# siyarvurucu/gym-macm

Hardware: AMD Instinct MI355X
Metric: agent·steps/sec, cm-flock-v0 64 agents × 4096 envs, at 1/2/4/8 MI355X (higher is better)
Workload: dtype f32; 1 GPU; cm-flock-v0 n_agents=[64] x 4096 envs per GPU, uniform random discrete actions (MultiDiscrete[3,3,3]) pre-generated on device, from reset (seed 0x6d61636d); envs_per_gpu=4096, n_agents=64, total_envs=4096, split=weak: 4096 envs per GPU, parallelism=env-sharded x1 (no data-path collective), obs=float32, max_contacts=2016, spill_slots=4096, launch=one macm_world_rollout_traj launch for the K timed steps, outputs=every step's ([K, E, N, ...] trajectory buffers)

## Files before the change

gym-macm_amd/csrc/flock_common.hpp:

```cpp
#pragma once

#include <hip/hip_runtime.h>
#include <stdint.h>

#include "../../include/macm.h"
#include "macm_math.h"

namespace macm {

constexpr float kEps = 1.1920928955078125e-07f;
constexpr float kLinearSlop = 0.005f;
constexpr float kAabbExtension = 0.1f;
constexpr float kAabbMultiplier = 2.0f;
constexpr float kMaxTranslation = 2.0f;
constexpr float kBaumgarte = 0.2f;
constexpr float kMaxLinearCorrection = 0.2f;
constexpr float kTimeToSleep = 0.5f;
constexpr float kLinearSleepTol = 0.01f;
constexpr float kPi32 = 3.14159265359f;

struct StepParams {
  int32_t n_envs, n_agents, n_targets, max_contacts;
  int32_t vel_iters, pos_iters, warm_starting;
  int32_t action_mode, reward_mode, coord;
  int32_t force_spill;
  int32_t sweep;
  float dt;
  float inv_dt;
  float inv_mass;
  float damp;
  float radius;
  float friction;
  float force_f32;
  double rot_step;
  double inv_hz;
  double force;
  double diag_c;
  double reward_radius;
  double time_limit;
};

struct WorldBuffers {
  float2* pos;
  float2* vel;
  float* angle;
  float4* fat;
  float* sleep;
  float2* targets;
// ... 126 lines not shown
  int2* listener;
  int32_t* winner;
  uint8_t* mask_out;
  double* health_out;
  uint8_t* alive_out;
  int32_t* winner_out;
  float4* snap_out;
};

__host__ __device__ inline int tdm_team_of(const TdmParams& T, int i) {
  int t = 0;
  while (t < T.n_teams - 1 && i >= T.team_end[t]) ++t;
  return t;
}

__device__ __forceinline__ void act_trig(float a, double* s0, double* c0, double* s1, double* c1) {
  if (fabsf(a) < 524288.0f) {
    macm_action_trig(a, s0, c0, s1, c1);
  } else {
    sincos((double)a, s0, c0);
    sincos((double)a + M_PI / 2, s1, c1);
  }
}

template <typename OT>
__device__ __forceinline__ double obs_sqrt(float x) {
  if constexpr (sizeof(OT) == 4) return (double)sqrtf(x);
  else return sqrt((double)x);
}

__device__ __forceinline__ float rcp_rn(float x) {
  const float y = __builtin_amdgcn_rcpf(x);
  const float e = __builtin_fmaf(-x, y, 1.0f);
// ... 144 lines not shown
```

gym-macm_amd/csrc/flock_rollout_ar_w64.hip:

```cpp
#define MACM_ROLLOUT_TU 1
#define MACM_AUTORESET_TU 1
#include "flock_step_w64.hip"
```

gym-macm_amd/csrc/flock_rollout_w64.hip:

```cpp
#define MACM_ROLLOUT_TU 1
#include "flock_step_w64.hip"
```

gym-macm_amd/csrc/flock_step_w64.hip:

```cpp
#include "bots.hpp"
#include "flock_common.hpp"
#include "flock_spill.hpp"
#include "tdm_obs.hpp"

namespace macm {

constexpr int W = 64;
constexpr int TCAP = 256;
constexpr int DEG = 16;
constexpr int ICAP = W / 2;
constexpr int RCH = 2;
constexpr int KREC = 4;
constexpr int KRECA = KREC;
constexpr int kLevelsMinIsland = 4;
constexpr int kPrio2T = 3;

#if defined(MACM_STAMPS) && !defined(MACM_TIMELINE)
#define STAMP(k)                                                                    \
  do {                                                                              \
    __builtin_amdgcn_s_waitcnt(0);                                                  \
    const unsigned long long _t = __builtin_amdgcn_s_memtime();                     \
    if (lane == 0) B.stamps[(size_t)e * 16 + (k)] = _t;                             \
  } while (0)
#define STAMP_STAT(k, v)                                                            \
// ... 62 lines not shown
  if (coord == MACM_COORD_CARTESIAN) {
    o[0] = (OT)r0;
    o[1] = (OT)cos(t0);
    o[2] = (OT)sin(t0);
    o[3] = (OT)r1;
    o[4] = (OT)cos(t1);
    o[5] = (OT)sin(t1);
  } else if constexpr (sizeof(OT) == 4) {
    st_g<kOut>(reinterpret_cast<float4*>(o), make_float4((float)r0, (float)t0, (float)r1, (float)t1));
  } else {
    st_g<kOut>(reinterpret_cast<double2*>(o), make_double2(r0, t0));
    st_g<kOut>(reinterpret_cast<double2*>(o) + 1, make_double2(r1, t1));
  }
}

template <typename OT>
__device__ __forceinline__ void write_obs(OT* o, int coord, float ang, float best, float rx, float ry, float tdx,
                                          float tdy, float td2) {
  const double t0 = wrap_pi(obs_atan2((double)ry, (double)rx) - (double)ang);
  const double t1 = wrap_pi(obs_atan2((double)tdy, (double)tdx) - (double)ang);
  write_obs_row(o, coord, obs_sqrt<OT>(best), t0, obs_sqrt<OT>(td2), t1);
}

typedef float pf2 __attribute__((ext_vector_type(2)));

__device__ __forceinline__ void warm_start_contact_pk(pf2& vA, pf2& vB, float nx, float ny, float ln, float ltg,
                                                      float mA, float mB) {
  const pf2 n = {nx, ny}, t = {ny, -nx};
  const pf2 P = ln * n + ltg * t;
  vA = vA - mA * P;
  vB = vB + mB * P;
}

__device__ __forceinline__ void solve_velocity_contact_pk(pf2& vA, pf2& vB, float nx, float ny, float& ln,
                                                          float& ltg, float mA, float mB, float kmass,
// ... 400 lines not shown
  }
  near2_min<2 * K, 32 + 2 * K, SCAL>(qa.x, qa.y, qb.x, qb.y, cme, st);
  near2_min<2 * K + 1, 33 + 2 * K, SCAL>(qa.z, qa.w, qb.z, qb.w, cme, st);
  if constexpr ((K & 1) == 1) __builtin_amdgcn_sched_barrier(0);
  if constexpr (K + 1 < 16) near2_step<K + 1, SCAL>(s_pc2, win, cme, st);
}

constexpr float kNearS = 1.0f;
constexpr int kNearCap = 12;
constexpr int kNearRetry = 8, kNearRetryMax = 64;
constexpr float kNearPad = 1.0f + 0x1p-18f;
constexpr float kNearMove2 = (kNearS * 0.25f) * (kNearS * 0.25f) * (1.0f - 0x1p-20f);
constexpr int kNearNone = 0, kNearValid = 1, kNearDense = 2;
constexpr int kNearCtlKeep = 1;
constexpr int kNearCtlPlain = 2;
constexpr int kNearKindPlain = 0, kNearKindList = 1, kNearKindRebuild = 2;

__device__ __forceinline__ void near_push(float d2, float thr2, uint32_t& mask) {
  asm volatile(
      "v_cmp_le_f32 vcc, %1, %2\n\t"
      "v_addc_co_u32 %0, vcc, %0, %0, vcc"
      : "+v"(mask)
      : "v"(d2), "v"(thr2)
      : "vcc");
}

__device__ __forceinline__ unsigned long long near_build(const float4* s_pc2, fvec2 cme, float thr2) {
  uint32_t lo = 0u, hi = 0u;
  float4 na = s_pc2[15], nb = s_pc2[31];
#pragma unroll 4
// ... 49 lines not shown
  return row;
}

__device__ __forceinline__ int write_new_pairs(int lane, unsigned long long newmask, uint32_t* ocab,
                                               float2* ocimp, int C, uint32_t* stage_ab = nullptr,
                                               float2* stage_im = nullptr) {
  const int cnt = __popcll(newmask);
  const int pre = wave_prefix_sum(cnt);
  const int total = __builtin_amdgcn_readlane(pre, W - 1);
  int w = total - pre;
  unsigned long long m = newmask;
  while (m) {
    const int j = 63 - __clzll(m);
    m &= ~(1ull << j);
    if (w < C) {
      st_g<kState>(ocab + w, (uint32_t)lane | ((uint32_t)j << 16));
      st_g<kState>(ocimp + w, make_float2(0.0f, 0.0f));
      if (stage_ab && w < RCH * W) {
        stage_ab[w] = (uint32_t)lane | ((uint32_t)j << 16);
        stage_im[w] = make_float2(0.0f, 0.0f);
      }
    }
    ++w;
  }
  return total;
}

struct TailObs {
  unsigned long long* ctl;
  unsigned int tag;
  int nsteps;
  int k;
  bool worker;
  bool more;
  int q, left;
// ... 84 lines not shown
  }
  __syncthreads();
}

struct StepCarry {
  bool valid;
  float2 p, v, tg;
  float ang, slp;
  float4 fat;
  uint32_t rab[RCH];
  float2 rim[RCH];
  uint32_t ar0, ar1;
  int M, step_count;
};

template <int MODE, int NCAP, typename OT, bool SCAL = false, bool CARRY = false, bool NEARL = false>
__device__ __attribute__((always_inline)) inline void step_w64_body(
    const StepParams& P, const WorldBuffers& B, const TdmParams& TP, const TdmBuffers& TB, int cur,
    const void* __restrict__ actions, OT* __restrict__ obs, int32_t* __restrict__ nbr_out,
    float* __restrict__ rew_out, uint8_t* __restrict__ coll_out, uint8_t* __restrict__ done_out,
    const int e = blockIdx.x, const int lane = threadIdx.x, TailObs* tl = nullptr, StepCarry* carry = nullptr,
    const void* actions_next = nullptr, void** pool_out = nullptr, const int near_ctl = 0) {
  constexpr bool kT = MODE == kTdm;
  static_assert(!CARRY || !kT, "the carried step is Flock's");
  static_assert(!NEARL || (!kT && NCAP == 64), "the candidate lists are the 64-record Flock sweep's");
#ifdef MACM_TIMELINE
  const unsigned long long tl_rt0 = __builtin_amdgcn_s_memrealtime(), tl_c0 = __builtin_amdgcn_s_memtime();
#endif
  const int N = P.n_agents;
  const int C = P.max_contacts;
  bool act = lane < N;
  const size_t ag = (size_t)e * N + lane;
  const int nxt = cur ^ 1;
  const unsigned long long lt = lanemask_lt(lane);

  __shared__ float2 s_c[W];
  __shared__ float2 s_v[W];
  constexpr int TMW = kT ? 1 : 2;
// ... 24 lines not shown
  static_assert(kT || sizeof(uint32_t) * 2 * 2 * W >= W * DEG, "s_adj must fit in s_tm");
  static_assert(sizeof(uint32_t) * 2 * TMW * W >= sizeof(float2) * W, "the level steps' dummy slots must fit in s_tm");
  __shared__ uint8_t s_ord[TCAP];
  __shared__ uint32_t s_cvis[TCAP / 32];
  __shared__ uint8_t s_deg[W], s_stack[W], s_ibodies[W], s_bisl[W];
  __shared__ uint16_t s_ic[ICAP + 1];
  __shared__ uint8_t s_ib[ICAP + 1];
  __shared__ uint8_t s_isolved[ICAP];
  __shared__ uint32_t s_imin[ICAP];
  __shared__ int s_nisl;
  __shared__ double s_hpd[W];
  __shared__ int8_t s_hit[W];
  __shared__ float s_ang[W];
  __shared__ uint4 s_nl[NEARL ? W : 1];
  __shared__ int s_nl_state, s_nl_retry;
#ifdef MACM_STAMPS
  __shared__ int s_stat_maxisl;
  int stat_near = 0;
#endif
  if constexpr (kT) {
    if (tl && tl->worker) {
      tdm_tail_row<OT>(P, B, TP, TB, obs, *tl, lane, s_c, s_ang, reinterpret_cast<float4*>(&s_pool),
                       tdm_obs_rb_stage_bytes(N) <= (int)sizeof(Pool));
      return;
    }
  }

  const uint32_t* cab = B.cab[cur] + (size_t)e * C;
  const float2* cimp = B.cimp[cur] + (size_t)e * C;
  bool carried = false;
// ... 113 lines not shown
  float ray_x = 0.0f, ray_y = 0.0f;
  if (act) {
    if (P.action_mode == MACM_ACTION_DISCRETE) {
      float af = (float)((double)ang + ((double)(a2 - 1) * P.rot_step) * P.inv_hz);
      double ad = (double)af;
      if (fabs(ad) > M_PI) {
        af = (float)(ad - sgn(ad) * (2.0 * M_PI));
        ad = (double)af;
      }
      ang = af;
      const double cc = ((a0 != 1) && (a1 != 1)) ? P.diag_c : 1.0;
      const double k0 = (double)(a0 - 1), k1 = (double)(a1 - 1);
      double force = P.force;
      if constexpr (kT) force = P.force * (1.0 - TP.percent_mov_penalty * (double)(cdm > 0.0));
      double s0, c0, s1, c1;
      act_trig(af, &s0, &c0, &s1, &c1);
      const double fx = (c0 * k0 + c1 * k1) * cc * force;
      const double fy = (s0 * k0 + s1 * k1) * cc * force;
      Fx = (float)fx;
      Fy = (float)fy;
      if constexpr (kT) {
        if (cda <= 0.0) {
          if (a3) {
            attacking = true;
            ray_x = p.x + (float)(TP.melee_range * c0);
            ray_y = p.y + (float)(TP.melee_range * s0);
            cda = TP.cooldown_atk;
            cdm = TP.cooldown_mov_penalty;
          }
        } else {
          cda -= P.inv_hz;
// ... 135 lines not shown
      if (TMW == 2 && T > 64) tmask1 = (unsigned long long)tm[2] | ((unsigned long long)tm[3] << 32);
      deg = __popcll(tmask) + __popcll(tmask1);
    }
  } else if (act) {
    for (int t = 0; t < T; ++t) {
      const uint32_t ab = s_tab[t];
      if ((int)(ab & 0xffffu) == lane || (int)(ab >> 16) == lane) {
        if (deg < DEG) s_adj[lane * DEG + deg] = (uint8_t)t;
        ++deg;
      }
    }
  }
  if constexpr (!kT) {
    if (touch_over || (!fast_dfs && __builtin_amdgcn_ballot_w64(deg > DEG) != 0ull) || P.force_spill) {
      if constexpr (CARRY) {
        if (carried) __builtin_amdgcn_fence(__ATOMIC_SEQ_CST, "workgroup");
        carry->valid = false;
      }
      if constexpr (NEARL) s_nl_state = kNearNone;
      spill::step_env<OT, true>(P, B, e, cur, actions, obs, nbr_out, rew_out, coll_out, done_out,
                                reinterpret_cast<unsigned char*>(&s_pool));
      return;
    }
  } else {
    if (touch_over || (!fast_dfs && __builtin_amdgcn_ballot_w64(deg > DEG) != 0ull) || P.force_spill) {
      __shared__ int s_slot;
      const int slot = spill::acquire_slot(B, e, &s_slot);
      if (slot < 0) {
        spill::keep_lists(P, B, e, cur);
        if (lane == 0) {
          B.status[e] |= MACM_ST_SPILL_WAIT;
// ... 691 lines not shown
      float4 win[kNearAhead];
#pragma unroll
      for (int k = 0; k < kNearAhead; ++k) win[k] = s_pc2[k];
      near_step<0, NCAP>(s_pc2, win, mk2(cx, cy), s1);
      best = s1.best;
      bj = s1.bj;
    }
  }
  const unsigned long long myov = moved_pairs(movedm, fn, lane) & valid & ~(1ull << lane);
  const unsigned long long oldm = (unsigned long long)s_oldm[2 * lane] | ((unsigned long long)s_oldm[2 * lane + 1] << 32);
  const bool coll = act && ((myov | oldm) != 0ull);
  const unsigned long long above = lane == 63 ? 0ull : (~0ull << (lane + 1));
  const unsigned long long newmask = act ? (myov & ~oldm & above) : 0ull;
  STAMP(10);

  if constexpr (CARRY) {
    if (lane == 0) {
      time_passed = B.time_passed[e];
      st_prev = B.status[e];
      const ulonglong2* ec = reinterpret_cast<const ulonglong2*>(B.env_counters + (size_t)e * 4);
      const ulonglong2 c01 = ec[0], c23 = ec[1];
      ctr[0] = c01.x;
      ctr[1] = c01.y;
      ctr[2] = c23.x;
      ctr[3] = c23.y;
    }
  }
  uint32_t* ocab = B.cab[nxt] + (size_t)e * C;
  float2* ocimp = B.cimp[nxt] + (size_t)e * C;
  uint32_t* const stage_ab = CARRY ? s_tab : nullptr;
  float2* const stage_im = CARRY ? reinterpret_cast<float2*>(s_tm) : nullptr;
  static_assert(sizeof(uint32_t) * RCH * W <= sizeof(s_pool.tab), "the staged entries must fit in s_tab");
  static_assert(!CARRY || sizeof(float2) * RCH * W <= sizeof(s_pool.tm), "the staged impulses must fit in s_tm");
  const int nnew = write_new_pairs(lane, newmask, ocab, ocimp, C, stage_ab, stage_im);
  int kept = 0, Tr = 0;
  for (int c = 0; c * W < M; ++c) {
    const int k = c * W + lane;
    uint32_t ab = 0u;
    if (c < RCH) {
#pragma unroll
      for (int q = 0; q < RCH; ++q)
// ... 5 lines not shown
    const bool touch = (tbits >> c) & 1u;
    if (k < M) {
      const int a = ab & 0xffffu, b = ab >> 16;
      keep = overlap(s_fn[a], s_fn[b]);
    }
    const unsigned long long mt = __ballot(touch), mk = __ballot(keep);
    const int trank = Tr + __popcll(mt & lt);
    const int krank = kept + __popcll(mk & lt);
    Tr += __popcll(mt);
    kept += __popcll(mk);
    if (keep) {
      const int w = nnew + krank;
      if (w < C) {
        float2 l = make_float2(0.0f, 0.0f);
        if (touch && trank < TCAP) l = make_float2(s_tln[trank], s_tlt[trank]);
        st_g<kState>(ocab + w, ab);
        st_g<kState>(ocimp + w, l);
        if constexpr (CARRY) {
          if (w < RCH * W) {
            stage_ab[w] = ab;
            stage_im[w] = l;
          }
        }
      }
    }
  }
  int total = nnew + kept;
  if (total > C) {
    status |= MACM_ST_CONTACT_OVERFLOW;
    total = C;
  }
  STAMP(11);

  float rew = 0.0f;
  if constexpr (!kT) {
    if (act) {
      const float tdx = tg.x - cx, tdy = tg.y - cy;
      const float td2 = tdx * tdx + tdy * tdy;
      const double d = sqrt((double)td2);
      if (coll) rew = -1.0f;
      else if (P.reward_mode == MACM_REWARD_LINEAR) rew = (float)((-d / 35) + 1);
      else rew = (d < P.reward_radius) ? 1.0f : 0.0f;
      st_g<kOut>(rew_out + ag, rew);
      if (coll_out) st_g<kOut>(coll_out + ag, (uint8_t)(coll ? 1 : 0));
      if (nbr_out) st_g<kOut>(nbr_out + ag, (int32_t)bj);
      if (obs) {
        const int od = P.coord == MACM_COORD_CARTESIAN ? 6 : 4;
        const float2 cn = s_c[bj];
        const float rx = cn.x - cx, ry = cn.y - cy;
        write_obs<OT>(obs + ag * od, P.coord, ang, best, rx, ry, tdx, tdy, td2);
      }
      st_g<kState>(B.pos + ag, make_float2(cx, cy));
      st_g<kState>(B.vel + ag, make_float2(vx, vy));
      st_g<kState>(B.angle + ag, ang);
      st_g<kState>(B.fat + ag, fn);
      st_g<kState>(B.sleep + ag, ns);
    }
  } else {
    if (lane < N) {
      if (act) {
        B.pos[ag] = make_float2(cx, cy);
        B.vel[ag] = make_float2(vx, vy);
        B.fat[ag] = fn;
        B.sleep[ag] = ns;
      }
      if (act0) {
        B.angle[ag] = ang;
        TB.cd_atk[ag] = cda;
        TB.cd_mov[ag] = cdm;
      }
      TB.health[ag] = hp;
// ... 31 lines not shown
  if constexpr (!kT) {
    c1 = __popcll(__ballot(act && coll));
    c2 = __popcll(__ballot(act && rew > 0.0f));
    if (P.reward_mode == MACM_REWARD_LINEAR) rsum = wave_pairwise_sum((double)rew);
  } else {
    c1 = __popcll(att_m);
    c2 = __popcll(alive0_m & ~livem);
    const int myteam = tdm_team_of(TP, lane);
    for (int t = 0; t < TP.n_teams; ++t)
      if (__ballot(act && myteam == t)) {
        ++alive_teams;
        last_team = t;
      }
  }
  if (lane == 0) {
    const double tp = time_passed + P.inv_hz;
    uint8_t dn = tp > P.time_limit ? 1 : 0;
    if constexpr (kT) {
      int win = win_prev;
      if (done_prev) dn = 1;
      if (alive_teams == 1) {
        dn = 1;
        win = last_team;
      }
      if (alive_teams == 0) dn = 1;
      TB.winner[e] = win;
      if (TB.winner_out) TB.winner_out[e] = win;
      TB.listener[e] = lis;
    }
    B.time_passed[e] = tp;
    B.done[e] = dn;
    if (done_out) done_out[e] = dn;
    B.step_count[e] = step_count + 1;
    B.ccount[nxt][e] = total;
    const int st = (mst1 ? 1 : 0) | (mst2 ? 2 : 0) | (mst4 ? 4 : 0);
    if (st) {
      B.status[e] = st_prev | st;
      report_status(B, st);
    }
    const unsigned long long c0 = kT ? (unsigned long long)__popcll(alive0_m) : (unsigned long long)N;
    ulonglong2* ec = reinterpret_cast<ulonglong2*>(B.env_counters + (size_t)e * 4);
    ec[0] = make_ulonglong2(ctr[0] + c0, ctr[1] + c1);
    ec[1] = make_ulonglong2(ctr[2] + c2, ctr[3] + (unsigned long long)dn);
    if constexpr (!kT) {
      if (P.reward_mode == MACM_REWARD_LINEAR) add_reward_sum(B, e, rsum);
    }
  }
  if constexpr (CARRY) {
    carry->p = make_float2(cx, cy);
    carry->v = make_float2(vx, vy);
    carry->ang = ang;
    carry->fat = fn;
    carry->slp = ns;
    carry->tg = tg;
    carry->M = total;
    carry->step_count = step_count + 1;
    __syncthreads();
#pragma unroll
    for (int c = 0; c < RCH; ++c) {
      const int k = c * W + lane;
      carry->rab[c] = 0u;
      carry->rim[c] = make_float2(0.0f, 0.0f);
      if (k < total) {
        carry->rab[c] = stage_ab[k];
        carry->rim[c] = stage_im[k];
      }
    }
    carry->valid = total <= RCH * W && !(mst1 | mst2 | mst4);
  }
  if constexpr (NEARL) {
    if (mst1 | mst2 | mst4) s_nl_state = kNearNone;
  }
  STAMP(13);
#ifdef MACM_TIMELINE
  {
    const unsigned long long rt1 = __builtin_amdgcn_s_memrealtime(), c1t = __builtin_amdgcn_s_memtime();
    const unsigned long long hw = (unsigned)__builtin_amdgcn_s_getreg((31 << 11) | 4);
    const unsigned long long xcc = (unsigned)__builtin_amdgcn_s_getreg((31 << 11) | 20);
    if (lane == 0) {
      unsigned long long* st = B.stamps + (size_t)e * 16;
// ... 229 lines not shown
    if constexpr (MODE == kTdm) {
      TB.mask_out = traj_row(TB.mask_out, kr, EN * (N - 1));
      TB.health_out = traj_row(TB.health_out, kr, EN);
      TB.alive_out = traj_row(TB.alive_out, kr, EN);
      TB.winner_out = traj_row(TB.winner_out, kr, (size_t)A.P.n_envs);
      TB.snap_out = A.tail_tag ? (k >= A.tail_k0 ? traj_row(TB.snap_out, (size_t)(k - A.tail_k0), EN) : nullptr)
                               : traj_row(TB.snap_out, kr, EN);
    }
    const size_t abytes = MODE == kTdm ? 4 : 3;
    uint8_t* const pol_in = A.policy_act ? A.policy_act + kr * EN * abytes : nullptr;
    __builtin_amdgcn_s_setprio(0);
    int sl = (int)threadIdx.x;
    if constexpr (MODE == kTdm) asm volatile("" : "+v"(sl));
    tl.k = k - A0.tail_k0;
    constexpr bool kNearL = MODE == kFlock && NCAP == 64;
    const int near_ctl = kNearL ? (k > 0 ? kNearCtlKeep : 0) | ((A.cur & kRollNearPlainBit) ? kNearCtlPlain : 0) : 0;
    if constexpr (CARRY) {
      const unsigned char* const act_k = static_cast<const unsigned char*>(A.actions) + (size_t)k * A.astride;
      step_w64_body<MODE, NCAP, OT, SCAL, true, kNearL>(
          A.P, A.B, A.TP, TB, (A.cur ^ k) & 1, act_k, obs, traj_row(A.nbr_out, kr, EN), traj_row(A.rew_out, kr, EN),
          traj_row(A.coll_out, kr, EN), traj_row(A.done_out, kr, (size_t)A.P.n_envs), env, sl, nullptr, &cy,
          k + 1 < ksteps ? act_k + A.astride : nullptr, nullptr, near_ctl);
      if (A.cur & kRollReloadBit) cy.valid = false;
      if (!cy.valid) __builtin_amdgcn_fence(__ATOMIC_SEQ_CST, "workgroup");
      __syncthreads();
    } else {
      step_w64_body<MODE, NCAP, OT, SCAL, false, kNearL>(
          A.P, A.B, A.TP, TB, kNearL ? (A.cur ^ k) & 1 : A.cur ^ (k & 1),
          pol_in ? pol_in : static_cast<const unsigned char*>(A.actions) + (size_t)k * A.astride, obs,
          traj_row(A.nbr_out, kr, EN), traj_row(A.rew_out, kr, EN), traj_row(A.coll_out, kr, EN),
          traj_row(A.done_out, kr, (size_t)A.P.n_envs), env, sl, MODE == kTdm ? &tl : nullptr, nullptr, nullptr, nullptr,
// ... 371 lines not shown
```

gym-macm_amd/csrc/macm_capi.hip:

```cpp
#include <math.h>
#include <stdio.h>
#include <string.h>

#include <algorithm>
#include <string>
#include <vector>

#include "flock_common.hpp"
#include "py_mt19937.hpp"

namespace macm {
hipError_t launch_step_w64(const StepParams& P, const WorldBuffers& B, int cur, const void* actions, void* obs,
                           bool obs_f64, int32_t* nbr, float* rew, uint8_t* coll, uint8_t* done, hipStream_t s);
hipError_t launch_rollout_w64(const StepParams& P, const WorldBuffers& B, int cur, const void* actions, void* obs,
                              bool obs_f64, int32_t* nbr, float* rew, uint8_t* coll, uint8_t* done, hipStream_t s,
                              int nsteps, unsigned long long astride, int traj, int reload);
hipError_t launch_init_w64(const StepParams& P, const WorldBuffers& B, int cur, void* obs, bool obs_f64,
                           int32_t* nbr, const uint8_t* mask, hipStream_t s);
hipError_t launch_observe_w64(const StepParams& P, const WorldBuffers& B, void* obs, bool obs_f64, int32_t* nbr,
                              hipStream_t s);
hipError_t launch_step_wg(const StepParams& P, const WorldBuffers& B, int cur, int tcap, const void* actions,
                          void* obs, bool obs_f64, int32_t* nbr, float* rew, uint8_t* coll, uint8_t* done,
                          hipStream_t s, HandoffStream* HS, uint8_t* bot_act = nullptr);
hipError_t launch_init_wg(const StepParams& P, const WorldBuffers& B, int cur, void* obs, bool obs_f64, int32_t* nbr,
// ... 383 lines not shown
  P.n_envs = n_envs;
  P.n_agents = N;
  P.n_targets = T;
  P.max_contacts = C;
  P.vel_iters = c.velocity_iterations;
  P.pos_iters = c.position_iterations;
  P.warm_starting = c.warm_starting ? 1 : 0;
  P.action_mode = c.action_mode;
  P.reward_mode = c.reward_mode;
  P.coord = c.coord;
  P.force_spill = 0;
  P.sweep = 0;
  fill_body_params(P, c.hz, c.radius, c.density, c.friction, c.linear_damping, c.agent_force,
                   c.agent_rotation_speed);
  P.reward_radius = c.reward_radius;
  P.time_limit = c.time_limit;

  WorldBuffers& B = w->B;
  memset(&B, 0, sizeof(B));
  const size_t EN = (size_t)n_envs * N;
  int rc = MACM_OK;
  if ((rc = dalloc(w, &B.pos, EN)) || (rc = dalloc(w, &B.vel, EN)) || (rc = dalloc(w, &B.angle, EN)) ||
      (rc = dalloc(w, &B.fat, EN)) || (rc = dalloc(w, &B.sleep, EN)) ||
      (rc = dalloc(w, &B.targets, (size_t)n_envs * T)) || (rc = dalloc(w, &B.tidx, (size_t)N)) ||
      (rc = dalloc(w, &B.ccount[0], (size_t)n_envs)) || (rc = dalloc(w, &B.ccount[1], (size_t)n_envs)) ||
      (rc = dalloc(w, &B.cab[0], (size_t)n_envs * C)) || (rc = dalloc(w, &B.cab[1], (size_t)n_envs * C)) ||
      (rc = dalloc(w, &B.cimp[0], (size_t)n_envs * C)) || (rc = dalloc(w, &B.cimp[1], (size_t)n_envs * C)) ||
      (rc = dalloc(w, &B.step_count, (size_t)n_envs)) || (rc = dalloc(w, &B.time_passed, (size_t)n_envs)) ||
      (rc = dalloc(w, &B.done, (size_t)n_envs)) || (rc = dalloc(w, &B.status, (size_t)n_envs)) ||
      (rc = dalloc(w, &B.env_counters, (size_t)n_envs * 4)) || (rc = dalloc(w, &B.env_rsum, (size_t)n_envs))
// ... 1418 lines not shown
```

gym-macm_amd/csrc/macm_math.h:

```cpp
#pragma once
#include <math.h>

#ifdef __HIPCC__
#define MACM_MATH_FN __device__ __forceinline__
#else
#define MACM_MATH_FN static inline
#endif

MACM_MATH_FN void macm_sincos(double x, double* sp, double* cp) {
  const double fn = rint(x * 6.36619772367581382433e-01);
  const int q = (int)fn;
  const double t1 = fma(-fn, 1.57079632673412561417e+00, x);
  const double w2 = fn * 6.07710050630396597660e-11;
  const double r2 = t1 - w2;
  const double e2 = (t1 - r2) - w2;
  const double tail = fma(-fn, 2.02226624879595063154e-21, e2);
  const double y0 = r2 + tail;
  const double y1 = (r2 - y0) + tail;
  const double z = y0 * y0;
  double ps = 1.58969099521155010221e-10;
  ps = fma(ps, z, -2.50507602534068634195e-08);
  ps = fma(ps, z, 2.75573137070700676789e-06);
  ps = fma(ps, z, -1.98412698298579493134e-04);
  ps = fma(ps, z, 8.33333333332248946124e-03);
  const double v = z * y0;
  const double s = y0 - ((z * (0.5 * y1 - v * ps) - y1) - v * -1.66666666666666324348e-01);
  double pc = -1.13596475577881948265e-11;
  pc = fma(pc, z, 2.08757232129817482790e-09);
  pc = fma(pc, z, -2.75573143513906633035e-07);
  pc = fma(pc, z, 2.48015872894767294178e-05);
  pc = fma(pc, z, -1.38888888888741095749e-03);
  pc = fma(pc, z, 4.16666666666666019037e-02);
  const double hz = 0.5 * z;
  const double wc = 1.0 - hz;
  const double c = wc + (((1.0 - wc) - hz) + (z * (z * pc) - y0 * y1));
  const int odd = q & 1;
  double so = odd ? c : s, co = odd ? s : c;
  if (q & 2) so = -so;
  if ((q + 1) & 2) co = -co;
  *sp = (x == 0.0) ? x : so;
  *cp = co;
}

MACM_MATH_FN void macm_sincos_pair(double x, double* s0p, double* c0p, double* s1p, double* c1p) {
  const double fn = rint(x * 6.36619772367581382433e-01);
  const int q = (int)fn;
  const double t1 = fma(-fn, 1.57079632673412561417e+00, x);
  const double w2 = fn * 6.07710050630396597660e-11;
  const double r2 = t1 - w2;
  const double e2 = (t1 - r2) - w2;
  const double tail = fma(-fn, 2.02226624879595063154e-21, e2);
  const double y0 = r2 + tail;
  const double y1 = (r2 - y0) + tail;
  const double P = 1.57079632679489655800e+00;
  const double x1 = x + P;
  const double bp = x1 - x;
  const double err = (x - (x1 - bp)) + (P - bp);
  const double y1b = y1 - (6.12323399573676603587e-17 + err);
  const double z = y0 * y0;
  double ps = 1.58969099521155010221e-10;
  ps = fma(ps, z, -2.50507602534068634195e-08);
  ps = fma(ps, z, 2.75573137070700676789e-06);
  ps = fma(ps, z, -1.98412698298579493134e-04);
  ps = fma(ps, z, 8.33333333332248946124e-03);
  const double v = z * y0;
  const double vs = v * -1.66666666666666324348e-01;
  const double vps = v * ps;
  const double sa = y0 - ((z * (0.5 * y1 - vps) - y1) - vs);
  const double sb = y0 - ((z * (0.5 * y1b - vps) - y1b) - vs);
  double pc = -1.13596475577881948265e-11;
  pc = fma(pc, z, 2.08757232129817482790e-09);
  pc = fma(pc, z, -2.75573143513906633035e-07);
  pc = fma(pc, z, 2.48015872894767294178e-05);
  pc = fma(pc, z, -1.38888888888741095749e-03);
  pc = fma(pc, z, 4.16666666666666019037e-02);
  const double hz = 0.5 * z;
  const double wc = 1.0 - hz;
  const double cz = ((1.0 - wc) - hz) + z * (z * pc);
  const double ca = wc + (cz - y0 * y1);
  const double cb = wc + (cz - y0 * y1b);
  const int odd = q & 1;
  double so = odd ? ca : sa, co = odd ? sa : ca;
  if (q & 2) so = -so;
  if ((q + 1) & 2) co = -co;
  const int q1 = q + 1;
  double so1 = odd ? sb : cb, co1 = odd ? cb : sb;
  if (q1 & 2) so1 = -so1;
  if ((q1 + 1) & 2) co1 = -co1;
  *s0p = (x == 0.0) ? x : so;
  *c0p = co;
  *s1p = so1;
  *c1p = co1;
}

#ifdef __cplusplus
#define MACM_MATH_TABLE static constexpr
#else
#define MACM_MATH_TABLE static const
#endif
#include "trig_fix.inc"

MACM_MATH_FN void macm_action_trig_raw(double x, double* s0, double* c0, double* s1, double* c1) {
  if (fabs(x) < 4.0) {
    macm_sincos_pair(x, s0, c0, s1, c1);
  } else {
    macm_sincos(x, s0, c0);
    macm_sincos(x + M_PI / 2, s1, c1);
  }
}

MACM_MATH_FN void macm_action_trig(float a, double* s0, double* c0, double* s1, double* c1) {
  macm_action_trig_raw((double)a, s0, c0, s1, c1);
  int hit = 0;
  for (int i = 0; i < MACM_TRIG_NNEAR; ++i) hit |= a == (float)kTrigFixNear[i][0];
  if (hit) {
    for (int i = 0; i < MACM_TRIG_NNEAR; ++i) {
      if (a == (float)kTrigFixNear[i][0]) {
        *s0 = kTrigFixNear[i][1]; *c0 = kTrigFixNear[i][2]; *s1 = kTrigFixNear[i][3]; *c1 = kTrigFixNear[i][4];
      }
    }
  }
  if (fabsf(a) >= 4.0f) {
    for (int i = 0; i < MACM_TRIG_NFAR; ++i) {
      if (a == (float)kTrigFixFar[i][0]) {
        *s0 = kTrigFixFar[i][1]; *c0 = kTrigFixFar[i][2]; *s1 = kTrigFixFar[i][3]; *c1 = kTrigFixFar[i][4];
      }
    }
  }
}

MACM_MATH_FN double obs_atan2_core(double ax, double ay) {
  const int swap = ay > ax;
  const double mx = swap ? ay : ax, mn = swap ? ax : ay;
  const int r0 = mn < 0.4375 * mx;
  const int r1 = !r0 && mn < 0.6875 * mx;
  const double ca = r1 ? 2.0 : 1.0, cb = r0 ? 0.0 : 1.0, cd = r0 ? 0.0 : 1.0;
  const double xr = fma(ca, mn, -(cb * mx)) / fma(cd, mn, ca * mx);
  const double z = xr * xr;
  double p = 1.62858201153657823623e-02;
  p = fma(p, z, -3.65315727442169155270e-02);
  p = fma(p, z, 4.97687799461593236017e-02);
  p = fma(p, z, -5.83357013379057348645e-02);
  p = fma(p, z, 6.66107313738753120669e-02);
  p = fma(p, z, -7.69187620504482999495e-02);
  p = fma(p, z, 9.09088713343650656196e-02);
  p = fma(p, z, -1.11111104054623557880e-01);
  p = fma(p, z, 1.42857142725034663711e-01);
  p = fma(p, z, -1.99999999998764832476e-01);
  p = fma(p, z, 3.33333333333329318027e-01);
  const double sz = z * p;
  const double hi = r1 ? 4.63647609000806093515e-01 : 7.85398163397448278999e-01;
  const double lo = r1 ? 2.26987774529616870924e-17 : 3.06161699786838301793e-17;
  double r = r0 ? fma(-xr, sz, xr) : hi - (fma(xr, sz, -lo) - xr);
  if (swap) r = (1.57079632679489655800e+00 - r) + 6.12323399573676603587e-17;
  return r;
}

MACM_MATH_FN double obs_atan2_finish(double r, double y, double x) {
  if (x < 0.0) r = (3.1415926535897931160e+00 - r) + 1.2246467991473531772e-16;
  if (x == 0.0 && y == 0.0) r = signbit(x) ? 3.1415926535897931160e+00 : 0.0;
  return copysign(r, y);
}

MACM_MATH_FN double obs_atan2(double y, double x) { return obs_atan2_finish(obs_atan2_core(fabs(x), fabs(y)), y, x); }
```

gym-macm_amd/csrc/rollout_autoreset.inc:

```

constexpr int kMtN = 624, kMtM = 397;

__device__ __forceinline__ uint32_t mt_temper(uint32_t y) {
  y ^= (y >> 11);
  y ^= (y << 7) & 0x9d2c5680u;
  y ^= (y << 15) & 0xefc60000u;
  y ^= (y >> 18);
  return y;
}

__device__ __forceinline__ uint32_t mt_mix(uint32_t hi, uint32_t lo, uint32_t src) {
  const uint32_t y = (hi & 0x80000000u) | (lo & 0x7fffffffu);
  return src ^ (y >> 1) ^ ((y & 1u) ? 0x9908b0dfu : 0u);
}

struct ResetLds {
  uint32_t mt[kMtN];
  uint32_t w[6 * W];
  float2 p[W];
  float a[W];
};

__device__ __forceinline__ void mt_twist_wave(uint32_t* s_mt, int lane) {
  const int lo[4] = {0, kMtN - kMtM, 2 * (kMtN - kMtM), kMtN - 1};
// ... 106 lines not shown
    OT* const obs = traj_row(A.obs, kr, EN * od);
    int32_t* const nbr = traj_row(A.nbr_out, kr, EN);
    TdmBuffers TB = A.TB;
    if constexpr (MODE == kTdm) {
      TB.mask_out = traj_row(TB.mask_out, kr, EN * (N - 1));
      TB.health_out = traj_row(TB.health_out, kr, EN);
      TB.alive_out = traj_row(TB.alive_out, kr, EN);
      TB.winner_out = traj_row(TB.winner_out, kr, (size_t)A.P.n_envs);
    }
    const size_t abytes = MODE == kTdm ? 4 : 3;
    uint8_t* const pol_in = A.policy_act ? A.policy_act + kr * EN * abytes : nullptr;
    __builtin_amdgcn_s_setprio(0);
    int sl = (int)threadIdx.x;
    if constexpr (MODE == kTdm) asm volatile("" : "+v"(sl));
    void* lds = nullptr;
    const int near_ctl = kNearL ? near_keep | ((A.cur & kRollNearPlainBit) ? kNearCtlPlain : 0) : 0;
    if constexpr (CARRY) {
      const unsigned char* const act_k = static_cast<const unsigned char*>(A.actions) + (size_t)k * A.astride;
      step_w64_body<MODE, NCAP, OT, SCAL, true, kNearL>(
          A.P, A.B, A.TP, TB, (A.cur ^ k) & 1, act_k, obs, nbr, traj_row(A.rew_out, kr, EN), traj_row(A.coll_out, kr, EN),
          traj_row(A.done_out, kr, (size_t)A.P.n_envs), env, sl, nullptr, &cy,
          k + 1 < nsteps ? act_k + A.astride : nullptr, &lds, near_ctl);
    } else {
      step_w64_body<MODE, NCAP, OT, SCAL, false, kNearL>(
          A.P, A.B, A.TP, TB, kNearL ? (A.cur ^ k) & 1 : A.cur ^ (k & 1),
          pol_in ? pol_in : static_cast<const unsigned char*>(A.actions) + (size_t)k * A.astride, obs, nbr,
          traj_row(A.rew_out, kr, EN), traj_row(A.coll_out, kr, EN), traj_row(A.done_out, kr, (size_t)A.P.n_envs), env, sl,
          nullptr, nullptr, nullptr, &lds, near_ctl);
    }
    int rl = (int)threadIdx.x;
    if constexpr (MODE == kTdm) asm volatile("" : "+v"(rl));
// ... 113 lines not shown
```

Baseline: 24.17 billion agent·steps/s.

## Skip per-step global state writeback in carried rollout; pin trig constants to SGPRs

```diff
diff --git a/gym-macm_amd/csrc/flock_common.hpp b/gym-macm_amd/csrc/flock_common.hpp
--- a/gym-macm_amd/csrc/flock_common.hpp
+++ b/gym-macm_amd/csrc/flock_common.hpp
@@ -32,6 +32,7 @@
   float radius;
   float friction;
   float force_f32;
+  float reward_thr2;
   double rot_step;
   double inv_hz;
   double force;
@@ -188,9 +189,10 @@
   return t;
 }
 
+template <bool KSPIN = false>
 __device__ __forceinline__ void act_trig(float a, double* s0, double* c0, double* s1, double* c1) {
   if (fabsf(a) < 524288.0f) {
-    macm_action_trig(a, s0, c0, s1, c1);
+    MACM_KS_FN(macm_action_trig, KSPIN)(a, s0, c0, s1, c1);
   } else {
     sincos((double)a, s0, c0);
     sincos((double)a + M_PI / 2, s1, c1);
diff --git a/gym-macm_amd/csrc/flock_rollout_ar_w64.hip b/gym-macm_amd/csrc/flock_rollout_ar_w64.hip
--- a/gym-macm_amd/csrc/flock_rollout_ar_w64.hip
+++ b/gym-macm_amd/csrc/flock_rollout_ar_w64.hip
@@ -1,3 +1,4 @@
 #define MACM_ROLLOUT_TU 1
+#define MACM_KS_SWITCH 1
 #define MACM_AUTORESET_TU 1
 #include "flock_step_w64.hip"
diff --git a/gym-macm_amd/csrc/flock_rollout_w64.hip b/gym-macm_amd/csrc/flock_rollout_w64.hip
--- a/gym-macm_amd/csrc/flock_rollout_w64.hip
+++ b/gym-macm_amd/csrc/flock_rollout_w64.hip
@@ -1,2 +1,3 @@
 #define MACM_ROLLOUT_TU 1
+#define MACM_KS_SWITCH 1
 #include "flock_step_w64.hip"
diff --git a/gym-macm_amd/csrc/flock_step_w64.hip b/gym-macm_amd/csrc/flock_step_w64.hip
--- a/gym-macm_amd/csrc/flock_step_w64.hip
+++ b/gym-macm_amd/csrc/flock_step_w64.hip
@@ -2,6 +2,12 @@
 #include "flock_common.hpp"
 #include "flock_spill.hpp"
 #include "tdm_obs.hpp"
+
+#ifdef MACM_KS_SWITCH
+#define MACM_KS_PIN_FLOCK true
+#else
+#define MACM_KS_PIN_FLOCK false
+#endif
 
 namespace macm {
 
@@ -100,11 +106,11 @@
   }
 }
 
-template <typename OT>
+template <typename OT, bool KSPIN = false>
 __device__ __forceinline__ void write_obs(OT* o, int coord, float ang, float best, float rx, float ry, float tdx,
                                           float tdy, float td2) {
-  const double t0 = wrap_pi(obs_atan2((double)ry, (double)rx) - (double)ang);
-  const double t1 = wrap_pi(obs_atan2((double)tdy, (double)tdx) - (double)ang);
+  const double t0 = wrap_pi(MACM_KS_FN(obs_atan2, KSPIN)((double)ry, (double)rx) - (double)ang);
+  const double t1 = wrap_pi(MACM_KS_FN(obs_atan2, KSPIN)((double)tdy, (double)tdx) - (double)ang);
   write_obs_row(o, coord, obs_sqrt<OT>(best), t0, obs_sqrt<OT>(td2), t1);
 }
 
@@ -535,6 +541,7 @@
 constexpr int kNearNone = 0, kNearValid = 1, kNearDense = 2;
 constexpr int kNearCtlKeep = 1;
 constexpr int kNearCtlPlain = 2;
+constexpr int kStepCtlWriteBack = 4;
 constexpr int kNearKindPlain = 0, kNearKindList = 1, kNearKindRebuild = 2;
 
 __device__ __forceinline__ void near_push(float d2, float thr2, uint32_t& mask) {
@@ -614,11 +621,12 @@
     const int j = 63 - __clzll(m);
     m &= ~(1ull << j);
     if (w < C) {
-      st_g<kState>(ocab + w, (uint32_t)lane | ((uint32_t)j << 16));
-      st_g<kState>(ocimp + w, make_float2(0.0f, 0.0f));
       if (stage_ab && w < RCH * W) {
         stage_ab[w] = (uint32_t)lane | ((uint32_t)j << 16);
         stage_im[w] = make_float2(0.0f, 0.0f);
+      } else {
+        st_g<kState>(ocab + w, (uint32_t)lane | ((uint32_t)j << 16));
+        st_g<kState>(ocimp + w, make_float2(0.0f, 0.0f));
       }
     }
     ++w;
@@ -733,6 +741,13 @@
   int M, step_count;
 };
 
+struct __align__(16) EnvCarry {
+  unsigned long long ctr[4];
+  double time_passed;
+  double rsum;
+  int status;
+};
+
 template <int MODE, int NCAP, typename OT, bool SCAL = false, bool CARRY = false, bool NEARL = false>
 __device__ __attribute__((always_inline)) inline void step_w64_body(
     const StepParams& P, const WorldBuffers& B, const TdmParams& TP, const TdmBuffers& TB, int cur,
@@ -741,6 +756,7 @@
     const int e = blockIdx.x, const int lane = threadIdx.x, TailObs* tl = nullptr, StepCarry* carry = nullptr,
     const void* actions_next = nullptr, void** pool_out = nullptr, const int near_ctl = 0) {
   constexpr bool kT = MODE == kTdm;
+  constexpr bool kPin = MACM_KS_PIN_FLOCK && !kT;
   static_assert(!CARRY || !kT, "the carried step is Flock's");
   static_assert(!NEARL || (!kT && NCAP == 64), "the candidate lists are the 64-record Flock sweep's");
 #ifdef MACM_TIMELINE
@@ -795,6 +811,7 @@
   __shared__ float s_ang[W];
   __shared__ uint4 s_nl[NEARL ? W : 1];
   __shared__ int s_nl_state, s_nl_retry;
+  __shared__ EnvCarry s_ec;
 #ifdef MACM_STAMPS
   __shared__ int s_stat_maxisl;
   int stat_near = 0;
@@ -938,7 +955,7 @@
       double force = P.force;
       if constexpr (kT) force = P.force * (1.0 - TP.percent_mov_penalty * (double)(cdm > 0.0));
       double s0, c0, s1, c1;
-      act_trig(af, &s0, &c0, &s1, &c1);
+      act_trig<kPin>(af, &s0, &c0, &s1, &c1);
       const double fx = (c0 * k0 + c1 * k1) * cc * force;
       const double fy = (s0 * k0 + s1 * k1) * cc * force;
       Fx = (float)fx;
@@ -1104,7 +1121,7 @@
   if constexpr (!kT) {
     if (touch_over || (!fast_dfs && __builtin_amdgcn_ballot_w64(deg > DEG) != 0ull) || P.force_spill) {
       if constexpr (CARRY) {
-        if (carried) __builtin_amdgcn_fence(__ATOMIC_SEQ_CST, "workgroup");
+        static_assert(RCH * W <= TCAP && RCH * W <= 64 * TMW, "a carried step must not need the spill step");
         carry->valid = false;
       }
       if constexpr (NEARL) s_nl_state = kNearNone;
@@ -1826,17 +1843,23 @@
   const unsigned long long newmask = act ? (myov & ~oldm & above) : 0ull;
   STAMP(10);
 
+  bool done_c = false;
   if constexpr (CARRY) {
     if (lane == 0) {
-      time_passed = B.time_passed[e];
-      st_prev = B.status[e];
-      const ulonglong2* ec = reinterpret_cast<const ulonglong2*>(B.env_counters + (size_t)e * 4);
-      const ulonglong2 c01 = ec[0], c23 = ec[1];
-      ctr[0] = c01.x;
-      ctr[1] = c01.y;
-      ctr[2] = c23.x;
-      ctr[3] = c23.y;
-    }
+      if (!carried) {
+        s_ec.time_passed = B.time_passed[e];
+        s_ec.status = B.status[e];
+        if (P.reward_mode == MACM_REWARD_LINEAR)
+          s_ec.rsum = __hip_atomic_load(B.env_rsum + e, __ATOMIC_RELAXED, __HIP_MEMORY_SCOPE_AGENT);
+        const ulonglong2* ec = reinterpret_cast<const ulonglong2*>(B.env_counters + (size_t)e * 4);
+        const ulonglong2 c01 = ec[0], c23 = ec[1];
+        s_ec.ctr[0] = c01.x;
+        s_ec.ctr[1] = c01.y;
+        s_ec.ctr[2] = c23.x;
+        s_ec.ctr[3] = c23.y;
+      }
+    }
+    done_c = __ballot(lane == 0 && s_ec.time_passed + P.inv_hz > P.time_limit) != 0ull;
   }
   uint32_t* ocab = B.cab[nxt] + (size_t)e * C;
   float2* ocimp = B.cimp[nxt] + (size_t)e * C;
@@ -1872,13 +1895,12 @@
       if (w < C) {
         float2 l = make_float2(0.0f, 0.0f);
         if (touch && trank < TCAP) l = make_float2(s_tln[trank], s_tlt[trank]);
-        st_g<kState>(ocab + w, ab);
-        st_g<kState>(ocimp + w, l);
-        if constexpr (CARRY) {
-          if (w < RCH * W) {
-            stage_ab[w] = ab;
-            stage_im[w] = l;
-          }
+        if (CARRY && w < RCH * W) {
+          stage_ab[w] = ab;
+          stage_im[w] = l;
+        } else {
+          st_g<kState>(ocab + w, ab);
+          st_g<kState>(ocimp + w, l);
         }
       }
     }
@@ -1888,6 +1910,10 @@
     status |= MACM_ST_CONTACT_OVERFLOW;
     total = C;
   }
+  bool wb = true;
+  if constexpr (CARRY)
+    wb = actions_next == nullptr || (near_ctl & kStepCtlWriteBack) || total > RCH * W || done_c ||
+         __ballot(status != 0) != 0ull;
   STAMP(11);
 
   float rew = 0.0f;
@@ -1895,10 +1921,9 @@
     if (act) {
       const float tdx = tg.x - cx, tdy = tg.y - cy;
       const float td2 = tdx * tdx + tdy * tdy;
-      const double d = sqrt((double)td2);
       if (coll) rew = -1.0f;
-      else if (P.reward_mode == MACM_REWARD_LINEAR) rew = (float)((-d / 35) + 1);
-      else rew = (d < P.reward_radius) ? 1.0f : 0.0f;
+      else if (P.reward_mode == MACM_REWARD_LINEAR) rew = (float)((-sqrt((double)td2) / 35) + 1);
+      else rew = (td2 < P.reward_thr2) ? 1.0f : 0.0f;
       st_g<kOut>(rew_out + ag, rew);
       if (coll_out) st_g<kOut>(coll_out + ag, (uint8_t)(coll ? 1 : 0));
       if (nbr_out) st_g<kOut>(nbr_out + ag, (int32_t)bj);
@@ -1906,13 +1931,15 @@
         const int od = P.coord == MACM_COORD_CARTESIAN ? 6 : 4;
         const float2 cn = s_c[bj];
         const float rx = cn.x - cx, ry = cn.y - cy;
-        write_obs<OT>(obs + ag * od, P.coord, ang, best, rx, ry, tdx, tdy, td2);
-      }
-      st_g<kState>(B.pos + ag, make_float2(cx, cy));
-      st_g<kState>(B.vel + ag, make_float2(vx, vy));
-      st_g<kState>(B.angle + ag, ang);
-      st_g<kState>(B.fat + ag, fn);
-      st_g<kState>(B.sleep + ag, ns);
+        write_obs<OT, kPin>(obs + ag * od, P.coord, ang, best, rx, ry, tdx, tdy, td2);
+      }
+      if (wb) {
+        st_g<kState>(B.pos + ag, make_float2(cx, cy));
+        st_g<kState>(B.vel + ag, make_float2(vx, vy));
+        st_g<kState>(B.angle + ag, ang);
+        st_g<kState>(B.fat + ag, fn);
+        st_g<kState>(B.sleep + ag, ns);
+      }
     }
   } else {
     if (lane < N) {
@@ -1974,6 +2001,7 @@
       }
   }
   if (lane == 0) {
+    if constexpr (CARRY) time_passed = s_ec.time_passed;
     const double tp = time_passed + P.inv_hz;
     uint8_t dn = tp > P.time_limit ? 1 : 0;
     if constexpr (kT) {
@@ -1988,21 +2016,42 @@
       if (TB.winner_out) TB.winner_out[e] = win;
       TB.listener[e] = lis;
     }
-    B.time_passed[e] = tp;
+    if constexpr (CARRY) {
+      st_prev = s_ec.status;
+#pragma unroll
+      for (int q = 0; q < 4; ++q) ctr[q] = s_ec.ctr[q];
+    }
+    if (wb) B.time_passed[e] = tp;
     B.done[e] = dn;
     if (done_out) done_out[e] = dn;
-    B.step_count[e] = step_count + 1;
-    B.ccount[nxt][e] = total;
+    if (wb) {
+      B.step_count[e] = step_count + 1;
+      B.ccount[nxt][e] = total;
+    }
     const int st = (mst1 ? 1 : 0) | (mst2 ? 2 : 0) | (mst4 ? 4 : 0);
     if (st) {
       B.status[e] = st_prev | st;
       report_status(B, st);
     }
     const unsigned long long c0 = kT ? (unsigned long long)__popcll(alive0_m) : (unsigned long long)N;
-    ulonglong2* ec = reinterpret_cast<ulonglong2*>(B.env_counters + (size_t)e * 4);
-    ec[0] = make_ulonglong2(ctr[0] + c0, ctr[1] + c1);
-    ec[1] = make_ulonglong2(ctr[2] + c2, ctr[3] + (unsigned long long)dn);
-    if constexpr (!kT) {
+    if (wb) {
+      ulonglong2* ec = reinterpret_cast<ulonglong2*>(B.env_counters + (size_t)e * 4);
+      ec[0] = make_ulonglong2(ctr[0] + c0, ctr[1] + c1);
+      ec[1] = make_ulonglong2(ctr[2] + c2, ctr[3] + (unsigned long long)dn);
+    }
+    if constexpr (CARRY) {
+      if (P.reward_mode == MACM_REWARD_LINEAR) {
+        const double racc = s_ec.rsum + rsum;
+        s_ec.rsum = racc;
+        if (wb) __hip_atomic_store(B.env_rsum + e, racc, __ATOMIC_RELAXED, __HIP_MEMORY_SCOPE_AGENT);
+      }
+      s_ec.time_passed = tp;
+      if (st) s_ec.status = st_prev | st;
+      s_ec.ctr[0] = ctr[0] + c0;
+      s_ec.ctr[1] = ctr[1] + c1;
+      s_ec.ctr[2] = ctr[2] + c2;
+      s_ec.ctr[3] = ctr[3] + (unsigned long long)dn;
+    } else if constexpr (!kT) {
       if (P.reward_mode == MACM_REWARD_LINEAR) add_reward_sum(B, e, rsum);
     }
   }
@@ -2024,6 +2073,10 @@
       if (k < total) {
         carry->rab[c] = stage_ab[k];
         carry->rim[c] = stage_im[k];
+        if (wb) {
+          st_g<kState>(ocab + k, carry->rab[c]);
+          st_g<kState>(ocimp + k, carry->rim[c]);
+        }
       }
     }
     carry->valid = total <= RCH * W && !(mst1 | mst2 | mst4);
@@ -2283,7 +2336,8 @@
     if constexpr (MODE == kTdm) asm volatile("" : "+v"(sl));
     tl.k = k - A0.tail_k0;
     constexpr bool kNearL = MODE == kFlock && NCAP == 64;
-    const int near_ctl = kNearL ? (k > 0 ? kNearCtlKeep : 0) | ((A.cur & kRollNearPlainBit) ? kNearCtlPlain : 0) : 0;
+    const int near_ctl = (kNearL ? (k > 0 ? kNearCtlKeep : 0) | ((A.cur & kRollNearPlainBit) ? kNearCtlPlain : 0) : 0) |
+                         (CARRY && (A.cur & kRollReloadBit) ? kStepCtlWriteBack : 0);
     if constexpr (CARRY) {
       const unsigned char* const act_k = static_cast<const unsigned char*>(A.actions) + (size_t)k * A.astride;
       step_w64_body<MODE, NCAP, OT, SCAL, true, kNearL>(
diff --git a/gym-macm_amd/csrc/macm_capi.hip b/gym-macm_amd/csrc/macm_capi.hip
--- a/gym-macm_amd/csrc/macm_capi.hip
+++ b/gym-macm_amd/csrc/macm_capi.hip
@@ -8,6 +8,7 @@
 
 #include "flock_common.hpp"
 #include "py_mt19937.hpp"
+#include "reward_threshold.h"
 
 namespace macm {
 hipError_t launch_step_w64(const StepParams& P, const WorldBuffers& B, int cur, const void* actions, void* obs,
@@ -421,6 +422,7 @@
   fill_body_params(P, c.hz, c.radius, c.density, c.friction, c.linear_damping, c.agent_force,
                    c.agent_rotation_speed);
   P.reward_radius = c.reward_radius;
+  P.reward_thr2 = macm_reward_thr2(c.reward_radius);
   P.time_limit = c.time_limit;
 
   WorldBuffers& B = w->B;
diff --git a/gym-macm_amd/csrc/macm_math.h b/gym-macm_amd/csrc/macm_math.h
--- a/gym-macm_amd/csrc/macm_math.h
+++ b/gym-macm_amd/csrc/macm_math.h
@@ -7,7 +7,22 @@
 #define MACM_MATH_FN static inline
 #endif
 
-MACM_MATH_FN void macm_sincos(double x, double* sp, double* cp) {
+#if defined(__HIPCC__) && defined(MACM_KS_SWITCH)
+template <bool KSPIN>
+__device__ __forceinline__ double macm_ks(double c) {
+  if constexpr (KSPIN) asm volatile("" : "+s"(c));
+  return c;
+}
+#define MACM_KS_TPL template <bool KSPIN = false>
+#define MACM_KS(c) macm_ks<KSPIN>(c)
+#define MACM_KS_FN(f, pin) f<pin>
+#else
+#define MACM_KS_TPL
+#define MACM_KS(c) (c)
+#define MACM_KS_FN(f, pin) f
+#endif
+
+MACM_KS_TPL MACM_MATH_FN void macm_sincos(double x, double* sp, double* cp) {
   const double fn = rint(x * 6.36619772367581382433e-01);
   const int q = (int)fn;
   const double t1 = fma(-fn, 1.57079632673412561417e+00, x);
@@ -18,19 +33,19 @@
   const double y0 = r2 + tail;
   const double y1 = (r2 - y0) + tail;
   const double z = y0 * y0;
-  double ps = 1.58969099521155010221e-10;
-  ps = fma(ps, z, -2.50507602534068634195e-08);
-  ps = fma(ps, z, 2.75573137070700676789e-06);
-  ps = fma(ps, z, -1.98412698298579493134e-04);
-  ps = fma(ps, z, 8.33333333332248946124e-03);
+  double ps = MACM_KS(1.58969099521155010221e-10);
+  ps = fma(ps, z, MACM_KS(-2.50507602534068634195e-08));
+  ps = fma(ps, z, MACM_KS(2.75573137070700676789e-06));
+  ps = fma(ps, z, MACM_KS(-1.98412698298579493134e-04));
+  ps = fma(ps, z, MACM_KS(8.33333333332248946124e-03));
   const double v = z * y0;
-  const double s = y0 - ((z * (0.5 * y1 - v * ps) - y1) - v * -1.66666666666666324348e-01);
-  double pc = -1.13596475577881948265e-11;
-  pc = fma(pc, z, 2.08757232129817482790e-09);
-  pc = fma(pc, z, -2.75573143513906633035e-07);
-  pc = fma(pc, z, 2.48015872894767294178e-05);
-  pc = fma(pc, z, -1.38888888888741095749e-03);
-  pc = fma(pc, z, 4.16666666666666019037e-02);
+  const double s = y0 - ((z * (0.5 * y1 - v * ps) - y1) - v * MACM_KS(-1.66666666666666324348e-01));
+  double pc = MACM_KS(-1.13596475577881948265e-11);
+  pc = fma(pc, z, MACM_KS(2.08757232129817482790e-09));
+  pc = fma(pc, z, MACM_KS(-2.75573143513906633035e-07));
+  pc = fma(pc, z, MACM_KS(2.48015872894767294178e-05));
+  pc = fma(pc, z, MACM_KS(-1.38888888888741095749e-03));
+  pc = fma(pc, z, MACM_KS(4.16666666666666019037e-02));
   const double hz = 0.5 * z;
   const double wc = 1.0 - hz;
   const double c = wc + (((1.0 - wc) - hz) + (z * (z * pc) - y0 * y1));
@@ -42,7 +57,7 @@
   *cp = co;
 }
 
-MACM_MATH_FN void macm_sincos_pair(double x, double* s0p, double* c0p, double* s1p, double* c1p) {
+MACM_KS_TPL MACM_MATH_FN void macm_sincos_pair(double x, double* s0p, double* c0p, double* s1p, double* c1p) {
   const double fn = rint(x * 6.36619772367581382433e-01);
   const int q = (int)fn;
   const double t1 = fma(-fn, 1.57079632673412561417e+00, x);
@@ -58,22 +73,22 @@
   const double err = (x - (x1 - bp)) + (P - bp);
   const double y1b = y1 - (6.12323399573676603587e-17 + err);
   const double z = y0 * y0;
-  double ps = 1.58969099521155010221e-10;
-  ps = fma(ps, z, -2.50507602534068634195e-08);
-  ps = fma(ps, z, 2.75573137070700676789e-06);
-  ps = fma(ps, z, -1.98412698298579493134e-04);
-  ps = fma(ps, z, 8.33333333332248946124e-03);
+  double ps = MACM_KS(1.58969099521155010221e-10);
+  ps = fma(ps, z, MACM_KS(-2.50507602534068634195e-08));
+  ps = fma(ps, z, MACM_KS(2.75573137070700676789e-06));
+  ps = fma(ps, z, MACM_KS(-1.98412698298579493134e-04));
+  ps = fma(ps, z, MACM_KS(8.33333333332248946124e-03));
   const double v = z * y0;
-  const double vs = v * -1.66666666666666324348e-01;
+  const double vs = v * MACM_KS(-1.66666666666666324348e-01);
   const double vps = v * ps;
   const double sa = y0 - ((z * (0.5 * y1 - vps) - y1) - vs);
   const double sb = y0 - ((z * (0.5 * y1b - vps) - y1b) - vs);
-  double pc = -1.13596475577881948265e-11;
-  pc = fma(pc, z, 2.08757232129817482790e-09);
-  pc = fma(pc, z, -2.75573143513906633035e-07);
-  pc = fma(pc, z, 2.48015872894767294178e-05);
-  pc = fma(pc, z, -1.38888888888741095749e-03);
-  pc = fma(pc, z, 4.16666666666666019037e-02);
+  double pc = MACM_KS(-1.13596475577881948265e-11);
+  pc = fma(pc, z, MACM_KS(2.08757232129817482790e-09));
+  pc = fma(pc, z, MACM_KS(-2.75573143513906633035e-07));
+  pc = fma(pc, z, MACM_KS(2.48015872894767294178e-05));
+  pc = fma(pc, z, MACM_KS(-1.38888888888741095749e-03));
+  pc = fma(pc, z, MACM_KS(4.16666666666666019037e-02));
   const double hz = 0.5 * z;
   const double wc = 1.0 - hz;
   const double cz = ((1.0 - wc) - hz) + z * (z * pc);
@@ -100,17 +115,17 @@
 #endif
 #include "trig_fix.inc"
 
-MACM_MATH_FN void macm_action_trig_raw(double x, double* s0, double* c0, double* s1, double* c1) {
+MACM_KS_TPL MACM_MATH_FN void macm_action_trig_raw(double x, double* s0, double* c0, double* s1, double* c1) {
   if (fabs(x) < 4.0) {
-    macm_sincos_pair(x, s0, c0, s1, c1);
+    MACM_KS_FN(macm_sincos_pair, KSPIN)(x, s0, c0, s1, c1);
   } else {
-    macm_sincos(x, s0, c0);
-    macm_sincos(x + M_PI / 2, s1, c1);
+    MACM_KS_FN(macm_sincos, KSPIN)(x, s0, c0);
+    MACM_KS_FN(macm_sincos, KSPIN)(x + M_PI / 2, s1, c1);
   }
 }
 
-MACM_MATH_FN void macm_action_trig(float a, double* s0, double* c0, double* s1, double* c1) {
-  macm_action_trig_raw((double)a, s0, c0, s1, c1);
+MACM_KS_TPL MACM_MATH_FN void macm_action_trig(float a, double* s0, double* c0, double* s1, double* c1) {
+  MACM_KS_FN(macm_action_trig_raw, KSPIN)((double)a, s0, c0, s1, c1);
   int hit = 0;
   for (int i = 0; i < MACM_TRIG_NNEAR; ++i) hit |= a == (float)kTrigFixNear[i][0];
   if (hit) {
@@ -129,7 +144,7 @@
   }
 }
 
-MACM_MATH_FN double obs_atan2_core(double ax, double ay) {
+MACM_KS_TPL MACM_MATH_FN double obs_atan2_core(double ax, double ay) {
   const int swap = ay > ax;
   const double mx = swap ? ay : ax, mn = swap ? ax : ay;
   const int r0 = mn < 0.4375 * mx;
@@ -137,17 +152,17 @@
   const double ca = r1 ? 2.0 : 1.0, cb = r0 ? 0.0 : 1.0, cd = r0 ? 0.0 : 1.0;
   const double xr = fma(ca, mn, -(cb * mx)) / fma(cd, mn, ca * mx);
   const double z = xr * xr;
-  double p = 1.62858201153657823623e-02;
-  p = fma(p, z, -3.65315727442169155270e-02);
-  p = fma(p, z, 4.97687799461593236017e-02);
-  p = fma(p, z, -5.83357013379057348645e-02);
-  p = fma(p, z, 6.66107313738753120669e-02);
-  p = fma(p, z, -7.69187620504482999495e-02);
-  p = fma(p, z, 9.09088713343650656196e-02);
-  p = fma(p, z, -1.11111104054623557880e-01);
-  p = fma(p, z, 1.42857142725034663711e-01);
-  p = fma(p, z, -1.99999999998764832476e-01);
-  p = fma(p, z, 3.33333333333329318027e-01);
+  double p = MACM_KS(1.62858201153657823623e-02);
+  p = fma(p, z, MACM_KS(-3.65315727442169155270e-02));
+  p = fma(p, z, MACM_KS(4.97687799461593236017e-02));
+  p = fma(p, z, MACM_KS(-5.83357013379057348645e-02));
+  p = fma(p, z, MACM_KS(6.66107313738753120669e-02));
+  p = fma(p, z, MACM_KS(-7.69187620504482999495e-02));
+  p = fma(p, z, MACM_KS(9.09088713343650656196e-02));
+  p = fma(p, z, MACM_KS(-1.11111104054623557880e-01));
+  p = fma(p, z, MACM_KS(1.42857142725034663711e-01));
+  p = fma(p, z, MACM_KS(-1.99999999998764832476e-01));
+  p = fma(p, z, MACM_KS(3.33333333333329318027e-01));
   const double sz = z * p;
   const double hi = r1 ? 4.63647609000806093515e-01 : 7.85398163397448278999e-01;
   const double lo = r1 ? 2.26987774529616870924e-17 : 3.06161699786838301793e-17;
@@ -162,4 +177,6 @@
   return copysign(r, y);
 }
 
-MACM_MATH_FN double obs_atan2(double y, double x) { return obs_atan2_finish(obs_atan2_core(fabs(x), fabs(y)), y, x); }
+MACM_KS_TPL MACM_MATH_FN double obs_atan2(double y, double x) {
+  return obs_atan2_finish(MACM_KS_FN(obs_atan2_core, KSPIN)(fabs(x), fabs(y)), y, x);
+}
diff --git a/gym-macm_amd/csrc/reward_threshold.h b/gym-macm_amd/csrc/reward_threshold.h
--- /dev/null
+++ b/gym-macm_amd/csrc/reward_threshold.h
@@ -0,0 +1,11 @@
+#pragma once
+#include <math.h>
+
+static inline float macm_reward_thr2(double R) {
+  if (!(R > 0.0)) return 0.0f;
+  if (isinf(R)) return INFINITY;
+  float T = (float)(R * R);
+  while (sqrt((double)T) < R) T = nextafterf(T, INFINITY);
+  while (T > 0.0f && sqrt((double)nextafterf(T, -INFINITY)) >= R) T = nextafterf(T, -INFINITY);
+  return T;
+}
diff --git a/gym-macm_amd/csrc/rollout_autoreset.inc b/gym-macm_amd/csrc/rollout_autoreset.inc
--- a/gym-macm_amd/csrc/rollout_autoreset.inc
+++ b/gym-macm_amd/csrc/rollout_autoreset.inc
@@ -144,7 +144,8 @@
     int sl = (int)threadIdx.x;
     if constexpr (MODE == kTdm) asm volatile("" : "+v"(sl));
     void* lds = nullptr;
-    const int near_ctl = kNearL ? near_keep | ((A.cur & kRollNearPlainBit) ? kNearCtlPlain : 0) : 0;
+    const int near_ctl = (kNearL ? near_keep | ((A.cur & kRollNearPlainBit) ? kNearCtlPlain : 0) : 0) |
+                         (CARRY && (A.cur & kRollReloadBit) ? kStepCtlWriteBack : 0);
     if constexpr (CARRY) {
       const unsigned char* const act_k = static_cast<const unsigned char*>(A.actions) + (size_t)k * A.astride;
       step_w64_body<MODE, NCAP, OT, SCAL, true, kNearL>(
```

Measured after the change: 24.89 billion agent·steps/s, median of 6. +3.0%, better.
